# Daniel-Lin-S/decode_tonal_langauge

Measured on AMD Instinct MI355X. Metric: mel-frames/sec (train step) SynthesisModelCNN, 128ch x 400t batch256, higher is better.
Workload: dtype f32; 1 GPU; SynthesisModelCNN 128ch x 400t -> 80 mel, 4 tones x 2 syllables, L=5, global batch 256 (strong scaling: 256 windows on rank 0), dropout 0.5, NAdam, 1,376,768,720 params; per_gpu_batch=256, global_batch=256, parallelism=dp1, init=drawn on every rank

## Files before the change

### decode_tonal_langauge_amd/csrc/tonal_wino63_epi.h

```cpp
#pragma once
#include "tonal_common.h"
#include "tonal_wino43_epi.h"
#include "tonal_wino43v_epi.h"

namespace tl {

__device__ __forceinline__ void v6_stamp(unsigned long long* st, int k) {
  if (st != nullptr) st[k] = __builtin_amdgcn_s_memtime();
}

#ifndef V6_ST_AUX
#define V6_ST_AUX 0
#endif
constexpr unsigned V6_DROP = 0x80000000u;
constexpr unsigned long long V6_HI = 0xffffffff00000000ull;

template <bool IMM>
__device__ __forceinline__ void v6_store_at(float x, __amdgpu_buffer_rsrc_t rs, unsigned vo, unsigned so, unsigned k) {
  if constexpr (IMM) __builtin_amdgcn_raw_buffer_store_b32(__builtin_bit_cast(unsigned, x), rs, vo + k, so, V6_ST_AUX);
  else __builtin_amdgcn_raw_buffer_store_b32(__builtin_bit_cast(unsigned, x), rs, vo, so + k, V6_ST_AUX);
}

__device__ __forceinline__ void v6_pair_swap(float& a, float& b) {
  const auto r = __builtin_amdgcn_permlane32_swap(__float_as_uint(a), __float_as_uint(b), false, false);
  a = __uint_as_float(r[0]);
  b = __uint_as_float(r[1]);
}

template <bool IMM>
__device__ __forceinline__ void v6_store_hex_pair(float (&ha)[8], float (&hb)[8], __amdgpu_buffer_rsrc_t rs, unsigned voAP, unsigned voAQ,
                                                  unsigned voBP, unsigned voBQ, unsigned so) {
#pragma unroll
  for (int i = 0; i < 8; ++i) v6_pair_swap(ha[i], hb[i]);
#pragma unroll
  for (int t = 0; t < 8; t += 2) {
    {
      const auto r = __builtin_amdgcn_permlane16_swap(__float_as_uint(ha[t]), __float_as_uint(ha[t + 1]), false, false);
      v6_store_at<IMM>(__uint_as_float(r[0]), rs, voAP, so, (unsigned)(t * 64));
      v6_store_at<IMM>(__uint_as_float(r[1]), rs, voAQ, so, (unsigned)(t * 64));
    }
    {
      const auto r = __builtin_amdgcn_permlane16_swap(__float_as_uint(hb[t]), __float_as_uint(hb[t + 1]), false, false);
      v6_store_at<IMM>(__uint_as_float(r[0]), rs, voBP, so, (unsigned)(t * 64));
      v6_store_at<IMM>(__uint_as_float(r[1]), rs, voBQ, so, (unsigned)(t * 64));
    }
  }
}
__device__ __forceinline__ unsigned v6_pair_offset(int colbase, int lr, int lh) {
  return (unsigned)((colbase >> 3) + ((lr >> 3) & 1)) * 512u + (unsigned)((lr >> 4) & 1) * 64u + (unsigned)lh * 32u + (unsigned)(lr & 7) * 4u;
}

__device__ __forceinline__ void wino63_rows(const f32x16 (&acc)[8], int e, float (&y)[6]) {
  const float m1 = acc[1][e], m2 = acc[2][e], m3 = acc[3][e], m4 = acc[4][e], m5 = acc[5][e], m6 = acc[6][e];
  const float a12 = m1 + m2, s12 = m1 - m2, a34 = m3 + m4, s34 = m3 - m4, a56 = m5 + m6, s56 = m5 - m6;
  y[0] = ((acc[0][e] + a12) + a34) + a56;
  y[1] = fmaf(0.5f, s56, fmaf(2.f, s34, s12));
  y[2] = fmaf(0.25f, a56, fmaf(4.f, a34, a12));
  y[3] = fmaf(0.125f, s56, fmaf(8.f, s34, s12));
  y[4] = fmaf(0.0625f, a56, fmaf(16.f, a34, a12));
  y[5] = fmaf(0.03125f, s56, fmaf(32.f, s34, s12)) + acc[7][e];
}
__device__ __forceinline__ void wino63_bt(const float (&d)[8], float (&v)[8]) {
  v[0] = fmaf(5.25f, d[2] - d[4], d[6] - d[0]);
  const float e1 = fmaf(-4.25f, d[4], d[2] + d[6]), o1 = fmaf(-4.25f, d[3], d[1] + d[5]);
  v[1] = e1 + o1;
  v[2] = e1 - o1;
  const float e2 = fmaf(0.25f, d[2], fmaf(-1.25f, d[4], d[6])), o2 = fmaf(0.5f, d[1], fmaf(-2.5f, d[3], 2.f * d[5]));
  v[3] = e2 + o2;
  v[4] = e2 - o2;
  const float e3 = fmaf(4.f, d[2], fmaf(-5.f, d[4], d[6])), o3 = fmaf(2.f, d[1], fmaf(-2.5f, d[3], 0.5f * d[5]));
  v[5] = e3 + o3;
  v[6] = e3 - o3;
  v[7] = fmaf(5.25f, d[3] - d[5], d[7] - d[1]);
}

__device__ __forceinline__ float selbit(uint32_t w, int j, float a, float b) {
  const uint32_t m = (uint32_t)__builtin_amdgcn_sbfe((int)w, j, 1);
  return __uint_as_float((__float_as_uint(a) & m) | (__float_as_uint(b) & ~m));
}

struct v6_rows {
  int tA, tB;
  long long seqA, seqB;
};
__device__ __forceinline__ v6_rows v6_rows_of(long long Hw, int Tp) {
  v6_rows r;
  const unsigned R = (unsigned)(6 * Hw);
  const unsigned s = R / (unsigned)Tp;
  r.seqA = (long long)(unsigned)__builtin_amdgcn_readfirstlane((int)s);
  r.tA = __builtin_amdgcn_readfirstlane((int)(R - s * (unsigned)Tp));
  r.tB = r.tA + 96;
  r.seqB = r.seqA;
  while (r.tB >= Tp) {
    r.tB -= Tp;
    ++r.seqB;
  }
  return r;
}
struct bits96 {
  unsigned long long lo;
  uint32_t hi;
};
__device__ __forceinline__ unsigned long long mask96(const bits96& a, const bits96& b, int j) {
  return j < 64 ? mask2l(a.lo, b.lo, j) : mask2(a.hi, b.hi, j - 64);
}
__device__ __forceinline__ bits96 v6_in_bits96(long long R0h, long long M) {
  bits96 r;
  r.lo = v5_in_bits<64, 1>(R0h, M);
  r.hi = (uint32_t)v5_in_bits<32, 1>(R0h + 64, M);
  return r;
}
__device__ __forceinline__ bits96 v6_valid_bits96(int t0, int Tp, int tlim, long long R0h, long long M) {
  bits96 r;
  r.lo = v5_valid_bits<64, 1>(t0, Tp, tlim, R0h, M);
  int t1 = t0 + 64;
  while (t1 >= Tp) t1 -= Tp;
  r.hi = (uint32_t)v5_valid_bits<32, 1>(t1, Tp, tlim, R0h + 64, M);
  return r;
}

template <bool VOUT, bool FULL>
__device__ __forceinline__ void v6_epilogue_pool(const tl_nt_params& p, const f32x16 (&acc)[8], const v5_pre_pool& pre, float* xch,
                                                 long long R0, int n0, int wm, int wn, int lr_in, int lh, long long tm,
                                                 unsigned long long* st = nullptr) {
  int lr = lr_in;
  asm volatile("" : "+v"(lr));
  const int colbase = n0 + wn * 32;
  const bool colok = colbase < p.N;
  const int col = colbase + lr;
  const long long Hw = tm * 128 + wm * 32;
  const int Tp = p.Tp, Tq = Tp >> 1;
  const v6_rows rw = v6_rows_of(Hw, Tp);
  const unsigned long long vA = v5_valid_bits<48, 2>(rw.tA, Tp, p.Tvalid, 6 * Hw, p.M);
  const unsigned long long vB = v5_valid_bits<48, 2>(rw.tB, Tp, p.Tvalid, 6 * Hw + 96, p.M);
  const float bv = pre.bv;
  const long long P0 = 3 * Hw;
  const long long prows = p.M >> 1;
  const int out_tp = (!VOUT && p.out_tp > 0) ? p.out_tp : Tq;
  const int tqa0 = rw.tA >> 1, tqb0 = rw.tB >> 1;
  const unsigned long long kA = v5_valid_bits<48, 1>(tqa0, Tq, out_tp, P0, prows);
  const unsigned long long kB = v5_valid_bits<48, 1>(tqb0, Tq, out_tp, P0 + 48, prows);
  const long long nseq = p.M / Tp;
  const long long obase = rw.seqA * out_tp;
  const __amdgpu_buffer_rsrc_t rsO = rsrc_of(!VOUT ? p.out + obase * (long long)p.ldo : nullptr,
                                            !VOUT ? (nseq * out_tp - obase) * (long long)p.ldo * 4 : 0);
  const unsigned ldo4 = (unsigned)p.ldo * 4u;
  const unsigned col4 = colok ? (unsigned)col * 4u : V6_DROP;
  int ta = tqa0, tb = tqb0;
  unsigned ra = (unsigned)tqa0 * ldo4, rb = ((unsigned)(rw.seqB - rw.seqA) * (unsigned)out_tp + (unsigned)tqb0) * ldo4;
  const unsigned seq_step = (unsigned)(out_tp - Tq) * ldo4;
  float pv[48];
  uint32_t wb0 = 0, wb1 = 0, ws0 = 0, ws1 = 0;
  v6_stamp(st, 8);
  static_for<0, 16>([&](auto E) {
    constexpr int e = decltype(E)::value;
    float y[6];
    wino63_rows(acc, e, y);
    unsigned vo_e = 0;
    if constexpr (!VOUT) vo_e = selmu(V6_HI, rb, ra) + col4;
    static_for<0, 3>([&](auto H) {
      constexpr int h = decltype(H)::value, j = 3 * e + h;
      const float y0 = lrelu01(y[2 * h] + bv, p.slope), y1 = lrelu01(y[2 * h + 1] + bv, p.slope);
      const bool valid = __builtin_amdgcn_inverse_ballot_w64(mask2l(vA, vB, j));
      const bool gt = (y1 > y0) && valid;
      const float o = valid ? (gt ? y1 : y0) : 0.f;
      pv[j] = o;
      if constexpr (j < 32) {
        wb0 = wb0 + wb0 + (uint32_t)gt;
        ws0 = ws0 + ws0 + (uint32_t)(o > 0.f);
      } else {
        wb1 = wb1 + wb1 + (uint32_t)gt;
        ws1 = ws1 + ws1 + (uint32_t)(o > 0.f);
      }
      if constexpr (!VOUT) {
        const unsigned vo = selmu(mask2l(kA, kB, j), vo_e, V5_OOB);
        __builtin_amdgcn_raw_buffer_store_b32(__builtin_bit_cast(unsigned, o), rsO, vo, (unsigned)h * ldo4, 0);
      }
    });
    if constexpr (!VOUT) {
      ta += 3;
      ra += 3u * ldo4;
      const bool wa = ta >= Tq;
      ta -= wa ? Tq : 0;
      ra += wa ? seq_step : 0u;
      tb += 3;
      rb += 3u * ldo4;
      const bool wbb = tb >= Tq;
      tb -= wbb ? Tq : 0;
      rb += wbb ? seq_step : 0u;
    }
  });
  v6_stamp(st, 9);
  {
    wb0 = bit_transpose32(__builtin_bitreverse32(wb0), lr);
    ws0 = bit_transpose32(__builtin_bitreverse32(ws0), lr);
    wb1 = bit_transpose32(__builtin_bitreverse32(wb1) >> 16, lr);
    ws1 = bit_transpose32(__builtin_bitreverse32(ws1) >> 16, lr);
    const long long wleft = (nseq * out_tp - obase) * (long long)p.ld_obits * 4;
    const long long wbase = obase * (long long)p.ld_obits + (colbase >> 5);
    const __amdgpu_buffer_rsrc_t rsB = rsrc_of(p.obits + wbase, wleft - (long long)(colbase >> 5) * 4);
    const __amdgpu_buffer_rsrc_t rsS = rsrc_of(p.osign ? p.osign + wbase : nullptr, p.osign ? wleft - (long long)(colbase >> 5) * 4 : 0);
    const unsigned t0h = (unsigned)(lh ? tqb0 : tqa0);
    const unsigned s0h = lh ? (unsigned)(rw.seqB - rw.seqA) : 0u;
#pragma unroll
    for (int b = 0; b < 2; ++b) {
      const unsigned r = 32u * b + (unsigned)lr;
      unsigned t = t0h + r;
      const unsigned c = t / (unsigned)Tq;
      t -= c * (unsigned)Tq;
      const bool keep = colok && r < 48u && t < (unsigned)out_tp && (P0 + 48 * lh + r) < prows;
      const unsigned wo = keep ? ((s0h + c) * (unsigned)out_tp + t) * (unsigned)p.ld_obits * 4u : V5_OOB;
      __builtin_amdgcn_raw_buffer_store_b32(b ? wb1 : wb0, rsB, wo, 0u, 0);
      __builtin_amdgcn_raw_buffer_store_b32(b ? ws1 : ws0, rsS, wo, 0u, 0);
    }
  }
  v6_stamp(st, 10);
  if constexpr (VOUT) {
    if (p.out != nullptr) {
      const __amdgpu_buffer_rsrc_t rsP = rsrc_of(p.out + P0 * (long long)p.ldo, (prows - P0) * (long long)p.ldo * 4);
      const unsigned pvoff = colok ? ((unsigned)(48 * lh) * (unsigned)p.ldo + (unsigned)col) * 4u : V5_OOB;
#pragma unroll
      for (int j = 0; j < 48; ++j) {
        const unsigned vo = selmu(mask2l(kA, kB, j), pvoff, V5_OOB);
        __builtin_amdgcn_raw_buffer_store_b32(__builtin_bit_cast(unsigned, pv[j]), rsP, vo, (unsigned)j * (unsigned)p.ldo * 4u, 0);
      }
    }
    const int slot = wm * 2 + lh;
    {
      float2 v2 = {pv[0], pv[1]};
      *reinterpret_cast<float2*>(xch + (slot * 64 + wn * 32 + lr) * 2) = v2;
    }
    __builtin_amdgcn_s_waitcnt(0xc07f);
    __builtin_amdgcn_s_barrier();
    asm volatile("" ::: "memory");
    v6_stamp(st, 11);
    float nb0 = 0.f, nb1 = 0.f;
    if (slot < 7) {
      const float2 v2 = *reinterpret_cast<const float2*>(xch + ((slot + 1) * 64 + wn * 32 + lr) * 2);
      nb0 = v2.x;
      nb1 = v2.y;
    }
    uint32_t seA = 0, seB = 0, nvA = 0, nvB = 0;
    {
      int t_a = tqa0, t_b = tqb0;
      const long long qa = (Hw >> 1), qb = (Hw >> 1) + 8;
      for (int k = 0; k < 8; ++k) {
        seA |= (uint32_t)(t_a == Tq - 6) << k;
        seB |= (uint32_t)(t_b == Tq - 6) << k;
        nvA |= (uint32_t)(FULL || qa + k < p.vout_quads) << k;
        nvB |= (uint32_t)(FULL || qb + k < p.vout_quads) << k;
        t_a += 6;
        if (t_a >= Tq) t_a -= Tq;
        t_b += 6;
        if (t_b >= Tq) t_b -= Tq;
      }
    }
    const long long Hn = Hw >> 1;
    const __amdgpu_buffer_rsrc_t rsV = rsrc_of(p.vout + Hn * 8 * (long long)p.ld_vout,
                                              (p.vout_quads - Hn) * 8 * (long long)p.ld_vout * 4);
    const unsigned pair4 = (unsigned)p.ld_vout * 64u;
    const unsigned offP = v6_pair_offset(colbase, lr, lh);
    const unsigned vvA = colok ? offP : V6_DROP, vvB = colok ? 4u * pair4 + offP : V6_DROP;
    const unsigned long long mraw = wm == 3 ? V6_HI : 0ull;
#pragma unroll
    for (int qp = 0; qp < 4; ++qp) {
      float vv[2][8];
#pragma unroll
      for (int hq = 0; hq < 2; ++hq) {
        const int q = 2 * qp + hq;
        const unsigned long long mend = mask2(seA, seB, q);
        float d[8];
#pragma unroll
        for (int k = 0; k < 6; ++k) d[k] = pv[6 * q + k];
        d[6] = selm(mend, 0.f, q < 7 ? pv[(6 * q + 6) % 48] : nb0);
        d[7] = selm(mend, 0.f, q < 7 ? pv[(6 * q + 7) % 48] : nb1);
        wino63_bt(d, vv[hq]);
        if (q == 7) {
#pragma unroll
          for (int k = 0; k < 6; ++k) vv[hq][k] = selm(mraw, d[k], vv[hq][k]);
        }
      }
      const int q = 2 * qp;
      const unsigned voA = selmu(mask2(nvA, nvA >> 1, q), vvA, V6_DROP), voB = selmu(mask2(nvB, nvB >> 1, q), vvB, V6_DROP);
      v6_store_hex_pair<FULL>(vv[0], vv[1], rsV, voA, voA + 1024u, voB, voB + 1024u, (unsigned)qp * pair4);
    }
    v6_stamp(st, 12);
    {
      const bool hw = wm == 0 && p.vhalo != nullptr;
      const __amdgpu_buffer_rsrc_t rsH = rsrc_of(hw ? p.vhalo + tm * 2 * (long long)p.N : nullptr, hw ? 2LL * p.N * 4 : 0);
      const unsigned ho = (colok && lh == 0) ? (unsigned)col * 4u : V5_OOB;
      __builtin_amdgcn_raw_buffer_store_b32(__builtin_bit_cast(unsigned, pv[0]), rsH, ho, 0u, 0);
      __builtin_amdgcn_raw_buffer_store_b32(__builtin_bit_cast(unsigned, pv[1]), rsH, ho, (unsigned)p.N * 4u, 0);
    }
  }
}

template <int EPI>
constexpr int v6_stores() {
  return EPI == W_EPI_POOL ? 52 : EPI == W_EPI_POOLV ? 70 : (EPI == W_EPI_MASK || EPI == W_EPI_LRELU) ? 96 : (EPI == W_EPI_MASKY || EPI == W_EPI_GY) ? 63 : 0;
}

struct v6_pre_mask {
  uint32_t s[3];
};
__device__ __forceinline__ v6_pre_mask v6_prefetch_mask(const tl_nt_params& p, long long R0, int n0, int wm, int wn, int lr, int lh) {
  const int colbase = n0 + wn * 32;
  const long long ra = R0 + wm * 192 + 96 * lh + lr;
  v6_pre_mask r = {{0u, 0u, 0u}};
#pragma unroll
  for (int k = 0; k < 3; ++k)
    if (colbase < p.N && ra + 32 * k < p.M) r.s[k] = p.auxbits[(ra + 32 * k) * (long long)p.ld_auxbits + (colbase >> 5)];
  return r;
}
template <bool FULL>
__device__ __forceinline__ void v6_epilogue_mask(const tl_nt_params& p, const f32x16 (&acc)[8], const v6_pre_mask& pre, long long R0,
                                                 int n0, int wm, int wn, int lr_in, int lh) {
  int lr = lr_in;
  asm volatile("" : "+v"(lr));
  const int colbase = n0 + wn * 32;
  const bool colok = colbase < p.N;
  const int col = colbase + lr;
  const long long Rw = R0 + wm * 192;
  const __amdgpu_buffer_rsrc_t rsO = rsrc_of(p.out + Rw * (long long)p.ldo, (p.M - Rw) * (long long)p.ldo * 4);
  const unsigned ovoff = colok ? ((unsigned)(96 * lh) * (unsigned)p.ldo + (unsigned)col) * 4u : V5_OOB;
  const unsigned ldo4 = (unsigned)p.ldo * 4u;
  bits96 inA = {~0ull, ~0u}, inB = inA;
  if (!FULL) {
    inA = v6_in_bits96(Rw, p.M);
    inB = v6_in_bits96(Rw + 96, p.M);
  }
  uint32_t sT[3];
#pragma unroll
  for (int k = 0; k < 3; ++k) sT[k] = bit_transpose32(pre.s[k], lr);
#pragma unroll
  for (int e = 0; e < 16; ++e) {
    float y[6];
    wino63_rows(acc, e, y);
#pragma unroll
    for (int h = 0; h < 6; ++h) {
      const int r = 6 * e + h;
      const float o = y[h] * selbit(sT[r >> 5], r & 31, 1.f, p.slope);
      const unsigned vo = FULL ? ovoff : selmu(mask96(inA, inB, r), ovoff, V5_OOB);
      __builtin_amdgcn_raw_buffer_store_b32(__builtin_bit_cast(unsigned, o), rsO, vo, (unsigned)r * ldo4, 0);
    }
  }
}

template <bool FULL>
__device__ __forceinline__ void v6_epilogue_lrelu(const tl_nt_params& p, const f32x16 (&acc)[8], const v5_pre_pool& pre, long long R0,
                                                  int n0, int wm, int wn, int lr_in, int lh) {
  int lr = lr_in;
  asm volatile("" : "+v"(lr));
  const int colbase = n0 + wn * 32;
  const bool colok = colbase < p.N;
  const int col = colbase + lr;
  const long long Rw = R0 + wm * 192;
  const __amdgpu_buffer_rsrc_t rsO = rsrc_of(p.out + Rw * (long long)p.ldo, (p.M - Rw) * (long long)p.ldo * 4);
  const unsigned ovoff = colok ? ((unsigned)(96 * lh) * (unsigned)p.ldo + (unsigned)col) * 4u : V5_OOB;
  const unsigned ldo4 = (unsigned)p.ldo * 4u;
  bits96 inA = {~0ull, ~0u}, inB = inA;
  if (!FULL) {
    inA = v6_in_bits96(Rw, p.M);
    inB = v6_in_bits96(Rw + 96, p.M);
  }
  const float bv = pre.bv;
#pragma unroll
  for (int e = 0; e < 16; ++e) {
    float y[6];
    wino63_rows(acc, e, y);
#pragma unroll
    for (int h = 0; h < 6; ++h) {
      const int r = 6 * e + h;
      const float o = lrelu01(y[h] + bv, p.slope);
      const unsigned vo = FULL ? ovoff : selmu(mask96(inA, inB, r), ovoff, V5_OOB);
      __builtin_amdgcn_raw_buffer_store_b32(__builtin_bit_cast(unsigned, o), rsO, vo, (unsigned)r * ldo4, 0);
    }
  }
}

struct v6_pre_masky {
  uint32_t s[3], a[3];
};
template <bool GTP = false>
__device__ __forceinline__ v6_pre_masky v6_prefetch_masky(const tl_nt_params& p, long long R0, int n0, int wm, int wn, int lr, int lh) {
  const int colbase = n0 + wn * 32;
  const long long ra = R0 + wm * 192 + 96 * lh + lr;
  v6_pre_masky r;
#pragma unroll
  for (int k = 0; k < 3; ++k) {
    r.s[k] = r.a[k] = 0u;
    if (colbase < p.N && ra + 32 * k < p.M) {
      long long row = ra + 32 * k;
      bool have = true;
      if constexpr (GTP) {
        const unsigned R = (unsigned)row, sq = R / (unsigned)p.Tp, t = R - sq * (unsigned)p.Tp;
        have = t < (unsigned)p.out_tp;
        row = (long long)sq * p.out_tp + t;
      }
      if (have) {
        r.s[k] = p.auxbits[row * (long long)p.ld_auxbits + (colbase >> 5)];
        r.a[k] = p.abits[row * (long long)p.ld_abits + (colbase >> 5)];
      }
    }
  }
  return r;
}
template <bool FULL, bool DIRECT = false>
__device__ __forceinline__ void v6_epilogue_masky(const tl_nt_params& p, const f32x16 (&acc)[8], const v6_pre_masky& pre, float* xch,
                                                  long long R0, int n0, int wm, int wn, int lr_in, int lh, long long tm,
                                                  unsigned long long* st = nullptr) {
  int lr = lr_in;
  asm volatile("" : "+v"(lr));
  const int colbase = n0 + wn * 32;
  const bool colok = colbase < p.N;
  const int col = colbase + lr;
  const long long Rw = R0 + wm * 192;
  const int Tp = p.Tp, hps = Tp / 3;
  const v6_rows rw = v6_rows_of(tm * 128 + wm * 32, Tp);
  uint32_t we[3], wo[3], sT[3], firstw = 0;
  {
    const bits96 okA = v6_valid_bits96(rw.tA, Tp, p.Tvalid_in >> 1, Rw, p.M);
    const bits96 okB = v6_valid_bits96(rw.tB, Tp, p.Tvalid_in >> 1, Rw + 96, p.M);
    const uint32_t okw[3] = {lh ? (uint32_t)okB.lo : (uint32_t)okA.lo, lh ? (uint32_t)(okB.lo >> 32) : (uint32_t)(okA.lo >> 32),
                             lh ? okB.hi : okA.hi};
    uint32_t fA = 0, fB = 0;
    int ha = rw.tA / 3, hb = rw.tB / 3;
    for (int k = 0; k < 32; ++k) {
      fA |= (uint32_t)(ha == 0) << k;
      fB |= (uint32_t)(hb == 0) << k;
      ha = ha + 1 == hps ? 0 : ha + 1;
      hb = hb + 1 == hps ? 0 : hb + 1;
    }
    firstw = lh ? fB : fA;
#pragma unroll
    for (int k = 0; k < 3; ++k) {
      sT[k] = bit_transpose32(pre.s[k], lr);
      const uint32_t aT = bit_transpose32(pre.a[k], lr);
      we[k] = okw[k] & ~aT;
      wo[k] = okw[k] & aT;
    }
  }
  const long long Hb = Rw / 3;
  const unsigned pair4 = (unsigned)p.ld_vout * 64u;
  const __amdgpu_buffer_rsrc_t rsY = rsrc_of(p.vout + Hb * 8 * (long long)p.ld_vout, (p.vout_quads - Hb) * 8 * (long long)p.ld_vout * 4);
  const __amdgpu_buffer_rsrc_t rsD = rsrc_of(p.vout2 + Hb * 8 * (long long)p.ld_vout, (p.vout_quads - Hb) * 8 * (long long)p.ld_vout * 4);
  const unsigned offP = v6_pair_offset(colbase, lr, lh);
  const unsigned vvA = colok ? offP : V6_DROP, vvB = colok ? 16u * pair4 + offP : V6_DROP;
  const int nexA = (int)(p.M / 3 - Hb < 64 ? p.M / 3 - Hb : 64) - lh, nexB = nexA - 32;
  float pe = 0.f, po = 0.f;
  float first_d[6], v1keep[8];
#pragma unroll
  for (int k = 0; k < 6; ++k) first_d[k] = 0.f;
#pragma unroll
  for (int k = 0; k < 8; ++k) v1keep[k] = 0.f;
  auto andf = [](float x, uint32_t m) { return __uint_as_float(__float_as_uint(x) & m); };
  v6_stamp(st, 8);
#pragma unroll
  for (int e = 0; e < 16; ++e) {
    if (e == 1) v6_stamp(st, 9);
    if (e == 4) v6_stamp(st, 10);
    if (e == 8) v6_stamp(st, 11);
    if (e == 12) v6_stamp(st, 12);
    float y[6];
    if constexpr (DIRECT) {
#pragma unroll
      for (int h = 0; h < 6; ++h) y[h] = acc[h][e];
    } else {
      wino63_rows(acc, e, y);
    }
    float dzr[12];
#pragma unroll
    for (int h = 0; h < 6; ++h) {
      const int r = 6 * e + h;
      const float t = y[h] * selbit(sT[r >> 5], r & 31, 1.f, p.slope);
      dzr[2 * h] = andf(t, (uint32_t)__builtin_amdgcn_sbfe((int)we[r >> 5], r & 31, 1));
      dzr[2 * h + 1] = andf(t, (uint32_t)__builtin_amdgcn_sbfe((int)wo[r >> 5], r & 31, 1));
    }
    float Yp[2][8], Vp[2][8];
#pragma unroll
    for (int hh = 0; hh < 2; ++hh) {
      const int j = 2 * e + hh;
      const float* d6 = dzr + 6 * hh;
      const float ev1 = (d6[0] + d6[2]) + d6[4], od1 = (d6[1] + d6[3]) + d6[5];
      const float ev2 = fmaf(16.f, d6[4], fmaf(4.f, d6[2], d6[0])), od2 = fmaf(32.f, d6[5], fmaf(8.f, d6[3], 2.f * d6[1]));
      const float ev3 = fmaf(0.0625f, d6[4], fmaf(0.25f, d6[2], d6[0])), od3 = fmaf(0.03125f, d6[5], fmaf(0.125f, d6[3], 0.5f * d6[1]));
      Yp[hh][0] = d6[0];
      Yp[hh][1] = ev1 + od1;
      Yp[hh][2] = ev1 - od1;
      Yp[hh][3] = ev2 + od2;
      Yp[hh][4] = ev2 - od2;
      Yp[hh][5] = ev3 + od3;
      Yp[hh][6] = ev3 - od3;
      Yp[hh][7] = d6[5];
      if (j == 0) {
#pragma unroll
        for (int k = 0; k < 6; ++k) first_d[k] = d6[k];
      } else {
        const uint32_t keep = ~(uint32_t)__builtin_amdgcn_sbfe((int)firstw, j, 1);
        float d[8];
        d[0] = andf(pe, keep);
        d[1] = andf(po, keep);
#pragma unroll
        for (int k = 0; k < 6; ++k) d[2 + k] = d6[k];
        wino63_bt(d, Vp[hh]);
      }
      pe = d6[4];
      po = d6[5];
    }
    {
      const int j = 2 * e;
      const unsigned so = (unsigned)e * pair4;
      const unsigned voA = FULL ? vvA : (j < nexA ? vvA : V6_DROP), voB = FULL ? vvB : (j < nexB ? vvB : V6_DROP);
      v6_store_hex_pair<FULL>(Yp[0], Yp[1], rsY, voA, voA + 1024u, voB, voB + 1024u, so);
      if (e == 0) {
#pragma unroll
        for (int i = 0; i < 8; ++i) v1keep[i] = Vp[1][i];
      } else {
        v6_store_hex_pair<FULL>(Vp[0], Vp[1], rsD, voA, voA + 1024u, voB, voB + 1024u, so);
      }
    }
    __builtin_amdgcn_sched_barrier(0);
  }
  v6_stamp(st, 13);
  const int slot = wm * 2 + lh;
  {
    float2 v2 = {pe, po};
    *reinterpret_cast<float2*>(xch + (slot * 64 + wn * 32 + lr) * 2) = v2;
  }
  __builtin_amdgcn_s_waitcnt(0xc07f);
  __builtin_amdgcn_s_barrier();
  asm volatile("" ::: "memory");
  {
    float fe = 0.f, fo = 0.f;
    if (slot > 0) {
      const float2 v2 = *reinterpret_cast<const float2*>(xch + ((slot - 1) * 64 + wn * 32 + lr) * 2);
      fe = v2.x;
      fo = v2.y;
    }
    const uint32_t keep = ~(uint32_t)__builtin_amdgcn_sbfe((int)firstw, 0, 1);
    float d[8], v[8];
    d[0] = andf(fe, keep);
    d[1] = andf(fo, keep);
#pragma unroll
    for (int k = 0; k < 6; ++k) d[2 + k] = first_d[k];
    wino63_bt(d, v);
    const bool raw = slot == 0;
#pragma unroll
    for (int k = 0; k < 8; ++k) v[k] = raw ? (k < 2 ? 0.f : d[k]) : v[k];
    const unsigned voA = FULL ? vvA : (0 < nexA ? vvA : V6_DROP), voB = FULL ? vvB : (0 < nexB ? vvB : V6_DROP);
    v6_store_hex_pair<FULL>(v, v1keep, rsD, voA, voA + 1024u, voB, voB + 1024u, 0u);
  }
  {
    const bool hw = wm == 3 && p.vhalo != nullptr;
    const __amdgpu_buffer_rsrc_t rsH = rsrc_of(hw ? p.vhalo + tm * 2 * (long long)p.N : nullptr, hw ? 2LL * p.N * 4 : 0);
    const unsigned ho = (colok && lh == 1) ? (unsigned)col * 4u : V5_OOB;
    __builtin_amdgcn_raw_buffer_store_b32(__builtin_bit_cast(unsigned, pe), rsH, ho, 0u, 0);
    __builtin_amdgcn_raw_buffer_store_b32(__builtin_bit_cast(unsigned, po), rsH, ho, (unsigned)p.N * 4u, 0);
  }
}

struct v6_pre_c1w {
  uint32_t s[3], c[3];
  f32x4 x[2];
};
__device__ __forceinline__ v6_pre_c1w v6_prefetch_c1w(const tl_nt_params& p, long long R0, int n0, int wm, int wn, int lr, int lh) {
  const int colbase = n0 + wn * 32;
  const long long rh = R0 + wm * 192 + 96 * lh;
  v6_pre_c1w r;
  const int Tp = p.Tp;
  const long long nseq = p.M / Tp;
  const unsigned s0 = (unsigned)(R0 / Tp);
  const __amdgpu_buffer_rsrc_t rsX = rsrc_of(p.c1x + (long long)s0 * p.c1T, (nseq - s0) * (long long)p.c1T * 4);
  typedef unsigned v4u __attribute__((ext_vector_type(4)));
#pragma unroll
  for (int k = 0; k < 3; ++k) {
    r.s[k] = r.c[k] = 0u;
    const long long rk = rh + lr + 32 * k;
    if (colbase < p.N && rk < p.M) {
      r.s[k] = p.auxbits[rk * (long long)p.ld_auxbits + (colbase >> 5)];
      r.c[k] = p.c1bits[rk * (long long)p.ld_auxbits + (colbase >> 5)];
    }
  }
  const unsigned Rx = (unsigned)(rh + 3 * lr), sx = Rx / (unsigned)Tp, tx = Rx - sx * (unsigned)Tp;
  const unsigned xo = ((sx - s0) * (unsigned)p.c1T + 2u * tx) * 4u;
  r.x[0] = __builtin_bit_cast(f32x4, (v4u)__builtin_amdgcn_raw_buffer_load_b128(rsX, xo, 0u, 0));
  r.x[1] = __builtin_bit_cast(f32x4, (v4u)__builtin_amdgcn_raw_buffer_load_b128(rsX, xo + 16u, 0u, 0));
  return r;
}
__device__ __forceinline__ void v6_epilogue_c1w(const tl_nt_params& p, const f32x16 (&acc)[8], const v6_pre_c1w& pre, float* xw,
                                                float* red, long long R0, int n0, int wm, int wn, int lr_in, int lh, long long tm) {
  int lr = lr_in;
  asm volatile("" : "+v"(lr));
  const int colbase = n0 + wn * 32;
  const bool colok = colbase < p.N;
  const int col = colbase + lr;
  const long long Hw = tm * 128 + wm * 32;
  const long long Rw = 6 * Hw;
  const int Tp = p.Tp;
  const v6_rows rw = v6_rows_of(Hw, Tp);
  const bits96 okA = v6_valid_bits96(rw.tA, Tp, p.Tvalid, Rw, p.M);
  const bits96 okB = v6_valid_bits96(rw.tB, Tp, p.Tvalid, Rw + 96, p.M);
  float* xh = xw + lh * 256;
  *reinterpret_cast<f32x4*>(xh + 8 * lr) = pre.x[0];
  *reinterpret_cast<f32x4*>(xh + 8 * lr + 4) = pre.x[1];
  c1w_acc ca;
  ca.clear();
  uint32_t sT[3], cT[3];
#pragma unroll
  for (int k = 0; k < 3; ++k) {
    sT[k] = bit_transpose32(pre.s[k], lr);
    cT[k] = bit_transpose32(pre.c[k], lr);
  }
  asm volatile("" ::: "memory");
#pragma unroll
  for (int e = 0; e < 16; ++e) {
    float y[6];
    wino63_rows(acc, e, y);
#pragma unroll
    for (int h = 0; h < 6; ++h) {
      const int r = 6 * e + h;
      const float2 xa = *reinterpret_cast<const float2*>(xh + 8 * (r / 3) + 2 * (r % 3));
      const float2 xb = *reinterpret_cast<const float2*>(xh + 8 * (r / 3) + 2 * (r % 3) + 2);
      const float dz = selm0(mask96(okA, okB, r), y[h] * selbit(sT[r >> 5], r & 31, 1.f, p.slope));
      const uint32_t am = (uint32_t)__builtin_amdgcn_sbfe((int)cT[r >> 5], r & 31, 1);
      auto pick = [am](float a, float b) { return __uint_as_float((__float_as_uint(a) & am) | (__float_as_uint(b) & ~am)); };
      ca.s[0] = fmaf(dz, pick(xa.y, xa.x), ca.s[0]);
      ca.s[1] = fmaf(dz, pick(xb.x, xa.y), ca.s[1]);
      ca.s[2] = fmaf(dz, pick(xb.y, xb.x), ca.s[2]);
      ca.b += dz;
    }
    __builtin_amdgcn_sched_barrier(0);
  }
  __syncthreads();
  c1w_reduce_store<4, 64>(p, red, ca, wm, wn * 32 + lr, lh, tm, col, colok);
}

}
```

Baseline: 1261 mel-frames/s.

## Use DPP quad transposes for 128-bit epilogue stores and hoist halo exchange

Replaces the permlane-swap based 32-bit scattered stores in the Winograd F(6,3) epilogue with a DPP 4x4 quad transpose, so each lane issues 128-bit buffer stores to a new offset layout. The cross-wave halo exchange through LDS and its barrier now happen before the main loop, using a recomputed last element. This lets the first tile's input transform be done inline instead of deferred to after the loop. The per-row first-window bitmask loop is also replaced by a closed-form shift-doubling construction. Removing the sched_barrier and adding extra DPP moves may change instruction scheduling and register pressure.

```diff
diff --git a/decode_tonal_langauge_amd/csrc/tonal_wino63_epi.h b/decode_tonal_langauge_amd/csrc/tonal_wino63_epi.h
--- a/decode_tonal_langauge_amd/csrc/tonal_wino63_epi.h
+++ b/decode_tonal_langauge_amd/csrc/tonal_wino63_epi.h
@@ -45,6 +45,39 @@
       v6_store_at<IMM>(__uint_as_float(r[1]), rs, voBQ, so, (unsigned)(t * 64));
     }
   }
+}
+template <class CTRL>
+__device__ __forceinline__ float v6_dpp(float x, CTRL) {
+  return __builtin_bit_cast(float, __builtin_amdgcn_mov_dpp(__builtin_bit_cast(int, x), CTRL::value, 0xf, 0xf, true));
+}
+__device__ __forceinline__ void v6_quad_transpose(float& v0, float& v1, float& v2, float& v3, bool odd, bool hi) {
+  using X1 = std::integral_constant<int, 0xB1>;
+  using X2 = std::integral_constant<int, 0x4E>;
+  auto stage = [](float& a, float& b, bool up, auto C) {
+    const float fa = v6_dpp(a, C), fb = v6_dpp(b, C);
+    a = up ? fb : a;
+    b = up ? b : fa;
+  };
+  stage(v0, v1, odd, X1{});
+  stage(v2, v3, odd, X1{});
+  stage(v0, v2, hi, X2{});
+  stage(v1, v3, hi, X2{});
+}
+template <bool IMM>
+__device__ __forceinline__ void v6_store_pair_x4(const float (&h0)[8], const float (&h1)[8], __amdgpu_buffer_rsrc_t rs, unsigned vo,
+                                                 unsigned so, bool odd, bool hi) {
+  typedef unsigned v4u __attribute__((ext_vector_type(4)));
+#pragma unroll
+  for (int g = 0; g < 4; ++g) {
+    float v0 = h0[2 * g], v1 = h1[2 * g], v2 = h0[2 * g + 1], v3 = h1[2 * g + 1];
+    v6_quad_transpose(v0, v1, v2, v3, odd, hi);
+    const v4u x = {__float_as_uint(v0), __float_as_uint(v1), __float_as_uint(v2), __float_as_uint(v3)};
+    if constexpr (IMM) __builtin_amdgcn_raw_buffer_store_b128(x, rs, vo + (unsigned)(g * 128), so, V6_ST_AUX);
+    else __builtin_amdgcn_raw_buffer_store_b128(x, rs, vo, so + (unsigned)(g * 128), V6_ST_AUX);
+  }
+}
+__device__ __forceinline__ unsigned v6_pair_offset_x4(int colbase, int lr) {
+  return (unsigned)((colbase >> 3) + (lr >> 3)) * 512u + (unsigned)(lr & 3) * 32u + (unsigned)((lr >> 2) & 1) * 16u;
 }
 __device__ __forceinline__ unsigned v6_pair_offset(int colbase, int lr, int lh) {
   return (unsigned)((colbase >> 3) + ((lr >> 3) & 1)) * 512u + (unsigned)((lr >> 4) & 1) * 64u + (unsigned)lh * 32u + (unsigned)(lr & 7) * 4u;
@@ -423,14 +456,15 @@
     const bits96 okB = v6_valid_bits96(rw.tB, Tp, p.Tvalid_in >> 1, Rw + 96, p.M);
     const uint32_t okw[3] = {lh ? (uint32_t)okB.lo : (uint32_t)okA.lo, lh ? (uint32_t)(okB.lo >> 32) : (uint32_t)(okA.lo >> 32),
                              lh ? okB.hi : okA.hi};
-    uint32_t fA = 0, fB = 0;
-    int ha = rw.tA / 3, hb = rw.tB / 3;
-    for (int k = 0; k < 32; ++k) {
-      fA |= (uint32_t)(ha == 0) << k;
-      fB |= (uint32_t)(hb == 0) << k;
-      ha = ha + 1 == hps ? 0 : ha + 1;
-      hb = hb + 1 == hps ? 0 : hb + 1;
-    }
+    uint32_t comb = 1u;
+#pragma unroll
+    for (int n = 1; n < 32; n *= 2) {
+      const unsigned s = (unsigned)(n * hps);
+      comb |= s < 32u ? comb << s : 0u;
+    }
+    const int hA = rw.tA / 3, hB = rw.tB / 3;
+    const int kA = hA == 0 ? 0 : hps - hA, kB = hB == 0 ? 0 : hps - hB;
+    const uint32_t fA = kA < 32 ? comb << kA : 0u, fB = kB < 32 ? comb << kB : 0u;
     firstw = lh ? fB : fA;
 #pragma unroll
     for (int k = 0; k < 3; ++k) {
@@ -444,16 +478,34 @@
   const unsigned pair4 = (unsigned)p.ld_vout * 64u;
   const __amdgpu_buffer_rsrc_t rsY = rsrc_of(p.vout + Hb * 8 * (long long)p.ld_vout, (p.vout_quads - Hb) * 8 * (long long)p.ld_vout * 4);
   const __amdgpu_buffer_rsrc_t rsD = rsrc_of(p.vout2 + Hb * 8 * (long long)p.ld_vout, (p.vout_quads - Hb) * 8 * (long long)p.ld_vout * 4);
-  const unsigned offP = v6_pair_offset(colbase, lr, lh);
-  const unsigned vvA = colok ? offP : V6_DROP, vvB = colok ? 16u * pair4 + offP : V6_DROP;
-  const int nexA = (int)(p.M / 3 - Hb < 64 ? p.M / 3 - Hb : 64) - lh, nexB = nexA - 32;
+  const unsigned vx = colok ? (unsigned)lh * 16u * pair4 + v6_pair_offset_x4(colbase, lr) : V6_DROP;
+  const int nexL = (int)(p.M / 3 - Hb < 64 ? p.M / 3 - Hb : 64) - 32 * lh - (lr & 1);
+  const bool qodd = (lr & 1) != 0, qhi = (lr & 2) != 0;
+  auto andf = [](float x, uint32_t m) { return __uint_as_float(__float_as_uint(x) & m); };
+  const int slot = wm * 2 + lh;
+  float fe = 0.f, fo = 0.f;
+  {
+    float y15;
+    if constexpr (DIRECT) {
+      y15 = acc[5][15];
+    } else {
+      float y[6];
+      wino63_rows(acc, 15, y);
+      y15 = y[5];
+    }
+    const float t = y15 * selbit(sT[2], 31, 1.f, p.slope);
+    float2 v2 = {andf(t, (uint32_t)__builtin_amdgcn_sbfe((int)we[2], 31, 1)), andf(t, (uint32_t)__builtin_amdgcn_sbfe((int)wo[2], 31, 1))};
+    *reinterpret_cast<float2*>(xch + (slot * 64 + wn * 32 + lr) * 2) = v2;
+  }
+  __builtin_amdgcn_s_waitcnt(0xc07f);
+  __builtin_amdgcn_s_barrier();
+  asm volatile("" ::: "memory");
+  if (slot > 0) {
+    const float2 v2 = *reinterpret_cast<const float2*>(xch + ((slot - 1) * 64 + wn * 32 + lr) * 2);
+    fe = v2.x;
+    fo = v2.y;
+  }
   float pe = 0.f, po = 0.f;
-  float first_d[6], v1keep[8];
-#pragma unroll
-  for (int k = 0; k < 6; ++k) first_d[k] = 0.f;
-#pragma unroll
-  for (int k = 0; k < 8; ++k) v1keep[k] = 0.f;
-  auto andf = [](float x, uint32_t m) { return __uint_as_float(__float_as_uint(x) & m); };
   v6_stamp(st, 8);
 #pragma unroll
   for (int e = 0; e < 16; ++e) {
@@ -492,17 +544,19 @@
       Yp[hh][5] = ev3 + od3;
       Yp[hh][6] = ev3 - od3;
       Yp[hh][7] = d6[5];
-      if (j == 0) {
-#pragma unroll
-        for (int k = 0; k < 6; ++k) first_d[k] = d6[k];
-      } else {
+      {
         const uint32_t keep = ~(uint32_t)__builtin_amdgcn_sbfe((int)firstw, j, 1);
         float d[8];
-        d[0] = andf(pe, keep);
-        d[1] = andf(po, keep);
+        d[0] = andf(j == 0 ? fe : pe, keep);
+        d[1] = andf(j == 0 ? fo : po, keep);
 #pragma unroll
         for (int k = 0; k < 6; ++k) d[2 + k] = d6[k];
         wino63_bt(d, Vp[hh]);
+        if (j == 0) {
+          const bool raw = slot == 0;
+#pragma unroll
+          for (int k = 0; k < 8; ++k) Vp[hh][k] = raw ? (k < 2 ? 0.f : d[k]) : Vp[hh][k];
+        }
       }
       pe = d6[4];
       po = d6[5];
@@ -510,46 +564,12 @@
     {
       const int j = 2 * e;
       const unsigned so = (unsigned)e * pair4;
-      const unsigned voA = FULL ? vvA : (j < nexA ? vvA : V6_DROP), voB = FULL ? vvB : (j < nexB ? vvB : V6_DROP);
-      v6_store_hex_pair<FULL>(Yp[0], Yp[1], rsY, voA, voA + 1024u, voB, voB + 1024u, so);
-      if (e == 0) {
-#pragma unroll
-        for (int i = 0; i < 8; ++i) v1keep[i] = Vp[1][i];
-      } else {
-        v6_store_hex_pair<FULL>(Vp[0], Vp[1], rsD, voA, voA + 1024u, voB, voB + 1024u, so);
-      }
-    }
-    __builtin_amdgcn_sched_barrier(0);
+      const unsigned vo = FULL ? vx : (j < nexL ? vx : V6_DROP);
+      v6_store_pair_x4<FULL>(Yp[0], Yp[1], rsY, vo, so, qodd, qhi);
+      v6_store_pair_x4<FULL>(Vp[0], Vp[1], rsD, vo, so, qodd, qhi);
+    }
   }
   v6_stamp(st, 13);
-  const int slot = wm * 2 + lh;
-  {
-    float2 v2 = {pe, po};
-    *reinterpret_cast<float2*>(xch + (slot * 64 + wn * 32 + lr) * 2) = v2;
-  }
-  __builtin_amdgcn_s_waitcnt(0xc07f);
-  __builtin_amdgcn_s_barrier();
-  asm volatile("" ::: "memory");
-  {
-    float fe = 0.f, fo = 0.f;
-    if (slot > 0) {
-      const float2 v2 = *reinterpret_cast<const float2*>(xch + ((slot - 1) * 64 + wn * 32 + lr) * 2);
-      fe = v2.x;
-      fo = v2.y;
-    }
-    const uint32_t keep = ~(uint32_t)__builtin_amdgcn_sbfe((int)firstw, 0, 1);
-    float d[8], v[8];
-    d[0] = andf(fe, keep);
-    d[1] = andf(fo, keep);
-#pragma unroll
-    for (int k = 0; k < 6; ++k) d[2 + k] = first_d[k];
-    wino63_bt(d, v);
-    const bool raw = slot == 0;
-#pragma unroll
-    for (int k = 0; k < 8; ++k) v[k] = raw ? (k < 2 ? 0.f : d[k]) : v[k];
-    const unsigned voA = FULL ? vvA : (0 < nexA ? vvA : V6_DROP), voB = FULL ? vvB : (0 < nexB ? vvB : V6_DROP);
-    v6_store_hex_pair<FULL>(v, v1keep, rsD, voA, voA + 1024u, voB, voB + 1024u, 0u);
-  }
   {
     const bool hw = wm == 3 && p.vhalo != nullptr;
     const __amdgpu_buffer_rsrc_t rsH = rsrc_of(hw ? p.vhalo + tm * 2 * (long long)p.N : nullptr, hw ? 2LL * p.N * 4 : 0);
```

Result: no change. 1260 mel-frames/s, median of 2 (-0.1%).
